# actionml/universal-recommender

Measured on NVIDIA H100. Metric: CCO train events/sec to indicator model, higher is better.
Workload: dtype int32+f64

## Files before the change

universal_recommender_b200/csrc/cco_api.cu:

```cuda
#include <cuda_runtime.h>
#include <dlfcn.h>
#include <stdarg.h>
#include <stdio.h>
#include <stdlib.h>
#include <string.h>

#include <algorithm>
#include <charconv>
#include <cmath>
#include <functional>
#include <cub/cub.cuh>
#include <nvtx3/nvToolsExt.h>
#include <condition_variable>
#include <mutex>
#include <string>
#include <thread>
#include <unordered_map>
#include <vector>

#include "../../include/cco_b200.h"
#include "cco_kernels.cuh"
#include "cco_sampler.cuh"
#include "cco_format.cuh"
#include "cco_strings.cuh"
// ... 518 lines not shown
    if (raw[i].n_rows > 0 && hist_fits_smem(c, raw[i].n_cols)) fit.push_back(i);
  for (size_t b0 = 0; b0 < fit.size(); b0 += kHistSegs) {
    const size_t b1 = std::min(fit.size(), b0 + kHistSegs);
    HistBatch hb{};
    long long nnz_sum = 0;
    int32_t max_cols = 0;
    for (size_t t = b0; t < b1; ++t) {
      nnz_sum += raw[fit[t]].nnz;
      max_cols = std::max(max_cols, raw[fit[t]].n_cols);
    }
    const size_t smem = ((size_t)max_cols + 1) / 2 * 4;
    const int per_sm = std::max(1, std::min<int>(2048 / kHistThreads, (int)(c->smem_optin / std::max<size_t>(smem + 1024, 1))));
    const long long target = (long long)c->sm_count * per_sm;
    for (size_t t = b0; t < b1; ++t) {
      const int i = fit[t];
      if (ready) CK(cudaStreamWaitEvent(s, ready[i], 0));
      const long long share = nnz_sum > 0 ? (target * raw[i].nnz + nnz_sum - 1) / nnz_sum : 1;
      const long long need = (raw[i].nnz + kHistMinEntries - 1) / kHistMinEntries;
      HistSeg &g = hb.seg[hb.n++];
      g.col = raw[i].col + raw[i].q_base;
      g.rp = raw[i].rp;
      g.nnz = raw[i].nnz;
      g.n_rows = raw[i].n_rows;
      g.q_lo = raw[i].q_base;
      g.q_hi = raw[i].q_base + raw[i].nnz;
      g.counts = counts + col_off[i];
      g.verdict = verdict ? verdict + 2 * i : nullptr;
      g.n_cols = raw[i].n_cols;
      g.cta0 = hb.cta_end;
      hb.cta_end += (int32_t)std::max(1LL, std::min(share, need));
    }
    CK(cudaFuncSetAttribute(k_col_counts_smem, cudaFuncAttributeMaxDynamicSharedMemorySize, (int)smem));
    k_col_counts_smem<<<hb.cta_end, kHistThreads, smem, s>>>(hb);
    c->launches++;
  }
  for (int i = 0; i < n_mats && copies; ++i) {
    if (raw[i].n_rows == 0 || hist_fits_smem(c, raw[i].n_cols)) continue;
    if (ready) CK(cudaStreamWaitEvent(s, ready[i], 0));
    int *v = verdict ? verdict + 2 * i : nullptr;
    if (v) {
      k_check_row_ptr<<<grid_for(raw[i].n_rows, 256, c->sm_count), 256, 0, s>>>(raw[i].n_rows, raw[i].rp, raw[i].q_base, raw[i].q_base + raw[i].nnz, v);
      c->launches++;
    }
    if (raw[i].nnz > 0) {
      k_col_histogram_flat<true><<<grid_for(raw[i].nnz, 256, c->sm_count), 256, 0, s>>>(raw[i].nnz, raw[i].col + raw[i].q_base, raw[i].n_cols,
                                                                                       counts + col_off[i], kHistCopies, copy_stride, v);
      c->launches++;
    }
  }
  if (copies) {
    k_sum_copies<<<grid_for(total_cols, 256, c->sm_count), 256, 0, s>>>(total_cols, kHistCopies, copy_stride, counts);
    c->launches++;
  }
  if (ready)
    for (int i = 0; i < n_mats; ++i) CK(cudaStreamWaitEvent(s, ready[i], 0));
  return CCO_OK;
}

static int nccl_check(int rc, const char *what) {
  if (rc != 0) return set_error(CCO_E_NCCL, "%s: %s", what, g_nccl.GetErrorString(rc));
  return CCO_OK;
}

static int downsample_all(cco_ctx *c, Arena &ar, const std::vector<DevRaw> &raw, const int *d_check , long long U,
                          const int32_t *raw_counts, int32_t *marg_all, const std::vector<long long> &col_off,
                          const cco_indicator_params_t *params, int32_t seed, uint32_t flags, std::vector<DevMat> &dm,
                          const cudaEvent_t *stage_ev ) {
  cudaStream_t s = c->stream;
  const int W = c->world, r = c->rank, n_mats = (int)raw.size();
  const long long S = (U + W - 1) / W;
  std::vector<uint32_t *> kept(n_mats, nullptr);
  std::vector<SampleScratch> sc(n_mats);
  for (int i = 0; i < n_mats; ++i) {
    DevMat *out = &dm[i];
    out->n_rows = U;
    out->n_cols = raw[i].n_cols;
    out->marg = marg_all + col_off[i];
    CKR(ar.alloc(&kept[i], (size_t)(W * S + 1)));
    CKR(ar.alloc(&out->rp, U + 1));
    CK(cudaMemsetAsync(kept[i], 0, sizeof(uint32_t) * (size_t)(W * S + 1), s));
    CKR(sample_scratch(c, ar, raw[i], raw_counts + col_off[i], params[i].max_interactions, &sc[i]));
    launch_count(c, raw[i], sc[i], params[i].max_interactions, seed, flags, d_check + 2 * i, kept[i], out->marg);
  }
  CK(cudaEventRecord(stage_ev[0], s));
  if (W > 1) {
    if (S > 0) {
      g_nccl.GroupStart();
      for (int i = 0; i < n_mats; ++i) {
        int rc = g_nccl.AllGather(kept[i] + (size_t)r * S, kept[i], (size_t)S, kNcclUint32, c->comm, s);
        if (rc != 0) { g_nccl.GroupEnd(); return nccl_check(rc, "ncclAllGather(kept counts)"); }
      }
      CKR(nccl_check(g_nccl.GroupEnd(), "ncclGroupEnd(kept counts)"));
    }
    if (col_off[n_mats] > 0)
      CKR(nccl_check(g_nccl.AllReduce(marg_all, marg_all, (size_t)col_off[n_mats], kNcclInt32, kNcclSum, c->comm, s), "ncclAllReduce(marginals)"));
  }
  std::vector<uint32_t> edge((size_t)n_mats * (W + 1), 0);
  for (int i = 0; i < n_mats; ++i) {
    CKR(exclusive_sum(c, ar, kept[i], dm[i].rp, U + 1));
    ar.release(kept[i]);
    if (W > 1)
      for (int q = 0; q <= W; ++q) CKR(mail_fetch(c, &edge[(size_t)i * (W + 1) + q], dm[i].rp + std::min<long long>((long long)q * S, U), 4));
  }
  CK(cudaEventRecord(stage_ev[1], s));
  if (W > 1) CKR(mail_wait(c));
  std::vector<long long> cap(n_mats, 0);
  std::vector<int32_t *> gathered(n_mats, nullptr);
  for (int i = 0; i < n_mats; ++i) {
    if (W == 1) {
      CKR(ar.alloc(&dm[i].col, std::max<long long>(raw[i].nnz, 1)));
      CKR(launch_write(c, ar, raw[i], sc[i], dm[i].col));
    } else {
      for (int q = 0; q < W; ++q) cap[i] = std::max<long long>(cap[i], (long long)edge[(size_t)i * (W + 1) + q + 1] - edge[(size_t)i * (W + 1) + q]);
      CKR(ar.alloc(&dm[i].col, std::max<long long>(edge[(size_t)i * (W + 1) + W], 1)));
      if (cap[i] > 0) {
        CKR(ar.alloc(&gathered[i], (size_t)(cap[i] * W)));
        CKR(launch_write(c, ar, raw[i], sc[i], gathered[i] + (size_t)r * cap[i]));
      }
    }
    ar.release(sc[i].col_thr);
    ar.release(sc[i].keep);
  }
  CK(cudaEventRecord(stage_ev[2], s));
  if (W > 1) {
    g_nccl.GroupStart();
    for (int i = 0; i < n_mats; ++i) {
      if (!gathered[i]) continue;
      int rc = g_nccl.AllGather(gathered[i] + (size_t)r * cap[i], gathered[i], (size_t)cap[i], kNcclInt32, c->comm, s);
      if (rc != 0) { g_nccl.GroupEnd(); return nccl_check(rc, "ncclAllGather(column blocks)"); }
    }
    CKR(nccl_check(g_nccl.GroupEnd(), "ncclGroupEnd(column blocks)"));
    for (int i = 0; i < n_mats; ++i) {
      if (!gathered[i]) continue;
      dim3 grid((unsigned)std::max(1, std::min(c->sm_count * 8 / W, 1024)), (unsigned)W);
      k_pack_blocks<<<grid, 256, 0, s>>>(W, S, U, cap[i], dm[i].rp, gathered[i], dm[i].col);
      c->launches++;
      ar.release(gathered[i]);
    }
  }
  CK(cudaEventRecord(stage_ev[3], s));
  CK(cudaGetLastError());
  return CCO_OK;
}


struct BinCfg {
  int group;
  int slots;
  int cap;
  int cbuf;
  int caux, keep_max, final_max;
  bool dense;
  bool bitmap;
  int bm_words;
  size_t region;
  size_t smem;
  int ctas_per_sm;
};

static int next_pow2(int x) {
  int p = 1;
  while (p < x) p <<= 1;
  return p;
}

template <int GROUP>
static int launch_rows_t(cco_ctx *c, const RowArgs &a, BinCfg &cfg, cudaStream_t st) {
  constexpr int CTA = GROUP == 32 ? 64 : GROUP;
  int occ = 1;
  void (*kern)(const RowArgs) = cfg.dense ? k_rows<GROUP, true> : k_rows<GROUP, false>;
  if constexpr (GROUP == 512 || GROUP == 256)
    if (cfg.bitmap) kern = k_rows<GROUP, false, true>;
  CK(cudaFuncSetAttribute(kern, cudaFuncAttributeMaxDynamicSharedMemorySize, (int)cfg.smem));
  CK(cudaOccupancyMaxActiveBlocksPerMultiprocessor(&occ, kern, CTA, cfg.smem));
  kern<<<c->sm_count * std::max(occ, 1) * 4, CTA, cfg.smem, st>>>(a);
  cfg.ctas_per_sm = occ;
  c->launches++;
  CK(cudaGetLastError());
  return CCO_OK;
}
static int launch_rows(cco_ctx *c, const RowArgs &a, BinCfg &cfg, cudaStream_t st) {
  switch (cfg.group) {
    case 1024: return launch_rows_t<1024>(c, a, cfg, st);
    case 512: return launch_rows_t<512>(c, a, cfg, st);
    case 256: return launch_rows_t<256>(c, a, cfg, st);
    case 128: return launch_rows_t<128>(c, a, cfg, st);
    case 32: return launch_rows_t<32>(c, a, cfg, st);
  }
  return set_error(CCO_E_INVALID_ARG, "internal: bad bin config");
}

static BinCfg make_cfg(cco_ctx *c, int group, int want_slots, int top_k, int n_cols_b) {
  BinCfg f;
  const int groups = group == 32 ? 2 : 1;
  f.group = group;
  f.final_max = next_pow2(top_k);
  f.cbuf = next_pow2(top_k + std::max(group, 128) + (group == 32 ? 64 : 0));
  if (group == 32 && top_k + 32 <= 96) f.cbuf = 128;
  f.keep_max = std::max(f.final_max, (f.cbuf - group) / 2);
  f.caux = group == 32 ? 0 : f.keep_max;
  size_t fixed = (size_t)(f.cbuf + f.caux) * 16 + 2 * 256 + 512 + 1024 + (size_t)(group / 32) * 256;
  size_t avail = (c->smem_optin - 1024) / groups;
  int max_slots = (int)((avail - fixed) / 4) & ~1023;
  f.slots = std::min(want_slots, max_slots);
  f.cap = f.slots / 2;
  f.dense = n_cols_b <= f.slots;
  f.bitmap = false;
  f.bm_words = 0;
  f.region = (fixed + (size_t)f.slots * 4 + 15) & ~(size_t)15;
  f.smem = f.region * groups;
  f.ctas_per_sm = 1;
  return f;
}

static bool use_bitmap(BinCfg &f, uint32_t max_w, int top_k, int n_cols_b) {
  if (f.dense || (f.group != 512 && f.group != 256)) return false;
  const long long seg = 32LL * (f.group / 32);
  const long long rep = (std::max<long long>(max_w, 64) + seg - 1) / seg * seg;
  const long long bm = ((long long)n_cols_b + 31) / 32;
  if (rep + bm + top_k > f.slots) return false;
  f.bitmap = true;
  f.slots = (int)rep;
  f.bm_words = (int)bm;
  return true;
}

static double llr_error_bound(long long n_users) {
  const double n = (double)n_users;
  return n > 1.0 ? std::ldexp(n * std::log(n), -47) : 0.0;
}
static bool cut_exact(long long n_users, int32_t max_marg_a, int32_t max_marg_b) {
  const double n = (double)n_users, r = (double)max_marg_a, c = (double)max_marg_b;
  if (r <= 0.0 || c <= 0.0) return true;
  double g = 2.0 / std::min(r * c, 0.5 * n);
  const double d = n - c - r + 1.0;
  if (d > 0.0) g = std::max(g, 2.0 * (1.0 / c - (r - 1.0) / d));
  return g > 2.0 * llr_error_bound(n_users);
}

struct IndicatorState {
  int mail_group = -1;
  long long rec[7] = {0, 0, 0, 0, 0, 0, 0};
  cudaEvent_t packed = nullptr;
  long long *out_ptr = nullptr;
  int32_t *p_col = nullptr, *p_cnt = nullptr;
  double *p_llr = nullptr;
  int32_t n_items_a = 0, n_cols_b = 0;
  bool emit_all = false;
};

static int enqueue_indicator(cco_ctx *c, Arena &ar, const uint32_t *at_ptr, const int32_t *at_users, int32_t n_items_a,
                             const int32_t *marg_a, int32_t max_marg_a, int32_t max_marg_b, const DevMat &B, long long n_users,
                             bool self, const cco_indicator_params_t &prm, uint32_t flags, bool emit_all, cudaEvent_t inputs_ready,
                             cudaEvent_t ev_begin, cudaEvent_t ev_end, IndicatorState *st) {
  cudaStream_t s = c->stream;
  const int32_t n_cols_b = B.n_cols;
  const int rank = c->rank, world = c->world;
  st->n_items_a = n_items_a;
  st->n_cols_b = n_cols_b;
  st->emit_all = emit_all;
  uint32_t *row_work, *masked, *sorted_work;
  unsigned long long *work64;
  long long *work_prefix;
  int32_t *ids, *rows_sorted, *d_pb = nullptr;
  size_t sort_tb = 0, order_tb = 0;
  if (n_items_a > 0)
    CK(cub::DeviceRadixSort::SortPairsDescending(nullptr, sort_tb, (const uint32_t *)nullptr, (uint32_t *)nullptr, (const int32_t *)nullptr,
                                                 (int32_t *)nullptr, n_items_a, 0, 32, s));
  int cb_bits = 1;
  while ((1LL << cb_bits) <= (long long)max_marg_b) ++cb_bits;
  cub::DoubleBuffer<uint32_t> order_cb(nullptr, nullptr);
  cub::DoubleBuffer<int32_t> order_id(nullptr, nullptr);
  if (n_cols_b > 0) CK(cub::DeviceRadixSort::SortPairs(nullptr, order_tb, order_cb, order_id, n_cols_b, 0, cb_bits, s));
  const bool beside = inputs_ready && ar.c && ((size_t)n_items_a + 1) * 8 <= Arena::kSlabMax && sort_tb <= Arena::kSlabMax &&
                      (size_t)n_cols_b * 4 <= Arena::kSlabMax && order_tb <= Arena::kSlabMax &&
                      ((size_t)max_marg_b + 2) * 4 <= Arena::kSlabMax;
  cudaStream_t ss = beside ? c->sched_stream : s;
  if (beside) CK(cudaStreamWaitEvent(ss, inputs_ready, 0));
  CKR(ar.alloc(&row_work, n_items_a + 1));
  CKR(ar.alloc(&masked, n_items_a + 1));
  CKR(ar.alloc(&work64, n_items_a + 1));
  CKR(ar.alloc(&work_prefix, n_items_a + 1));
  CKR(ar.alloc(&ids, n_items_a + 1));
  CKR(ar.alloc(&sorted_work, n_items_a + 1));
  CKR(ar.alloc(&rows_sorted, n_items_a + 1));
  CK(cudaMemsetAsync(work64 + n_items_a, 0, 8, ss));
  k_row_work<<<grid_for((long long)n_items_a * kSG, 256, c->sm_count), 256, 0, ss>>>(n_items_a, at_ptr, at_users, B.rp,
                                                                                  row_work, work64, ids, nullptr);
  c->launches++;
  CKR(exclusive_sum(c, ar, (const long long *)work64, work_prefix, (long long)n_items_a + 1, ss));
  if (world > 1) {
    CKR(ar.alloc(&d_pb, world + 1));
    k_partition_rows<<<1, ((world + 1 + 31) / 32) * 32, 0, ss>>>(work_prefix, n_items_a, world, d_pb);
    c->launches++;
  }
  k_mask_work<<<grid_for(n_items_a, 256, c->sm_count), 256, 0, ss>>>(n_items_a, row_work, d_pb, rank, masked);
  c->launches++;
  if (n_items_a > 0) {
    void *tmp;
    CKR(ar.alloc((char **)&tmp, sort_tb));
    CK(cub::DeviceRadixSort::SortPairsDescending(tmp, sort_tb, masked, sorted_work, ids, rows_sorted, n_items_a, 0, 32, ss));
    ar.release(tmp);
  }
  const int k_eff = emit_all ? 1 : prm.top_k;
  const bool warp_ok = k_eff + 32 <= 256;
  struct BinSpec { int group, slots; uint32_t max_w; };
  std::vector<BinSpec> spec = {{1024, 1 << 20, 0xffffffffu}, {1024, 1 << 20, 0xffffffffu}, {512, 16384, 8192u}, {256, 8192, 4096u}};
  if (warp_ok) {
    spec.push_back({128, 4096, 2048u});
    spec.push_back({32, 2048, 1024u});
    spec.push_back({32, 1024, 512u});
    spec.push_back({32, 512, 256u});
  } else {
    spec.push_back({128, 4096, 2048u});
  }
  const int kBins = (int)spec.size();
  std::vector<BinCfg> cfgs(kBins);
  for (int b = 0; b < kBins; ++b) cfgs[b] = make_cfg(c, spec[b].group, spec[b].slots, k_eff, n_cols_b);
  BinCfg &cfgL = cfgs[1];
  int key_bits = 1;
  while (((1LL << key_bits) - 1) <= (long long)n_cols_b) ++key_bits;
  int count_bits = 32 - key_bits;
  const long long k11_max = std::min<long long>(max_marg_a, max_marg_b);
  if (count_bits < 1 || k11_max >= (1LL << count_bits))
    return set_error(CCO_E_UNSUPPORTED,
                     "co-occurrence counts up to %lld over %d columns do not fit the packed 32-bit accumulator word "
                     "(key %d bits + count %d bits): lower maxItemsPerUser/maxEventsPerEventType for this event type "
                     "(\"Limits\" in include/cco_b200.h)", k11_max, n_cols_b, key_bits, count_bits);
  std::vector<uint32_t> h_thr(kBins);
  for (int b = 0; b < kBins; ++b) {
    const BinCfg &f = cfgs[std::min(b + 1, kBins - 1)];
    uint32_t lim = b + 1 < kBins ? spec[b + 1].max_w : 0u;
    if (b + 1 < kBins && !f.dense) lim = std::min<uint32_t>(lim, (uint32_t)f.cap);
    h_thr[b] = lim;
    if (b > 0) h_thr[b] = std::min(h_thr[b], h_thr[b - 1]);
  }
  const bool bitmap_ok = !emit_all && cut_exact(n_users, max_marg_a, max_marg_b) &&
                         2ull * (unsigned long long)std::max(max_marg_a, 0) * (unsigned long long)std::max(max_marg_b, 0) <
                             (unsigned long long)n_users;
  for (int b = 1; b < kBins && bitmap_ok; ++b) use_bitmap(cfgs[b], h_thr[b - 1], k_eff, n_cols_b);
  int32_t *d_bounds;
  CKR(ar.alloc(&d_bounds, kBins + 3));
  BinThresholds bt;
  memset(&bt, 0, sizeof bt);
  for (int b = 0; b < kBins; ++b) bt.t[b] = h_thr[b];
  k_bin_bounds<<<1, 32, 0, ss>>>(n_items_a, sorted_work, kBins, bt, d_bounds);
  c->launches++;
  int32_t *key_of_col, *first_key_of_cb, *order_id0, *order_id1;
  uint32_t *order_cb0, *order_cb1;
  const int32_t n_order = std::max<int32_t>(n_cols_b, 1);
  CKR(ar.alloc(&key_of_col, n_order));
  CKR(ar.alloc(&first_key_of_cb, (size_t)max_marg_b + 2));
  CKR(ar.alloc(&order_cb0, n_order));
  CKR(ar.alloc(&order_cb1, n_order));
  CKR(ar.alloc(&order_id0, n_order));
  CKR(ar.alloc(&order_id1, n_order));
  order_cb = cub::DoubleBuffer<uint32_t>(order_cb0, order_cb1);
  order_id = cub::DoubleBuffer<int32_t>(order_id0, order_id1);
  if (n_cols_b > 0) {
    k_col_order_init<<<grid_for(n_cols_b, 256, c->sm_count, 4), 256, 0, ss>>>(n_cols_b, B.marg, order_cb0, order_id0);
    void *tmp;
    CKR(ar.alloc((char **)&tmp, order_tb));
    CK(cub::DeviceRadixSort::SortPairs(tmp, order_tb, order_cb, order_id, n_cols_b, 0, cb_bits, ss));
    ar.release(tmp);
    k_col_order<<<grid_for(n_cols_b, 256, c->sm_count, 4), 256, 0, ss>>>(n_cols_b, max_marg_b, order_cb.Current(), order_id.Current(),
                                                                        key_of_col, first_key_of_cb);
    k_relabel_cols<<<c->sm_count * 8, 256, 0, ss>>>(B.rp + B.n_rows, key_of_col, B.col);
    c->launches += 3;
  }
  const int32_t *marg_key = reinterpret_cast<const int32_t *>(order_cb.Current()), *col_of_key = order_id.Current();
  if (beside) {
    cudaEvent_t scheduled;
    CKR(pooled_event(c, false, &scheduled));
    CK(cudaEventRecord(scheduled, ss));
    CK(cudaStreamWaitEvent(s, scheduled, 0));
  }
  ColTerm *col_terms;
  CKR(ar.alloc(&col_terms, std::max<int32_t>(n_cols_b, 1)));
  if (n_cols_b > 0) {
    k_col_terms<<<grid_for(n_cols_b, 256, c->sm_count, 4), 256, 0, s>>>(n_cols_b, marg_key, col_of_key, n_users, flags, col_terms);
    c->launches++;
  }
  int32_t stride = emit_all ? n_cols_b : std::min<int32_t>(prm.top_k, n_cols_b);
  if (stride < 1) stride = 1;
  int32_t *o_col, *o_cnt, *o_len;
  double *o_llr = nullptr;
  unsigned long long *d_distinct;
  int *d_err;
  size_t cells = (size_t)std::max(n_items_a, 1) * stride;
  CKR(ar.alloc(&o_col, cells));
  CKR(ar.alloc(&o_cnt, cells));
  if (!emit_all) CKR(ar.alloc(&o_llr, cells));
  CKR(ar.alloc(&o_len, n_items_a + 1));
  CKR(ar.alloc(&d_distinct, 2));
  CKR(ar.alloc(&d_err, 1));
  CK(cudaMemsetAsync(o_len, 0, sizeof(int32_t) * ((size_t)n_items_a + 1), s));
  CK(cudaMemsetAsync(d_distinct, 0, 16, s));
  CK(cudaMemsetAsync(d_err, 0, 4, s));
  RowArgs a;
  memset(&a, 0, sizeof a);
  a.at_ptr = at_ptr;
  a.at_users = at_users;
  a.b_ptr = B.rp;
  a.b_col = B.col;
  a.marg_a = marg_a;
  a.marg_b = marg_key;
  a.key_of_col = key_of_col;
  a.first_key_of_cb = first_key_of_cb;
  a.key_shift = 0;
  while (((long long)std::max(n_cols_b - 1, 0) >> a.key_shift) >= kCutBins) ++a.key_shift;
  a.max_marg_b = max_marg_b;
  a.col_terms = col_terms;
  a.rows_sorted = rows_sorted;
  a.row_work = row_work;
  a.bin_bounds = d_bounds;
  a.n_cols_b = n_cols_b;
  a.n_users = n_users;
  a.self = self ? 1 : 0;
  a.top_k = k_eff;
  a.has_min_llr = prm.has_min_llr;
  a.min_llr = prm.min_llr;
  a.cut_ok = cut_exact(n_users, max_marg_a, max_marg_b) ? 1 : 0;
  a.llr_eps2 = 2.0 * llr_error_bound(n_users);
  a.flags = flags;
  a.count_bits = count_bits;
  a.out_stride = stride;
  a.out_col = o_col;
  a.out_llr = o_llr;
  a.out_cnt = o_cnt;
  a.out_len = o_len;
  a.stat_distinct = d_distinct;
  a.stat_evaluated = d_distinct + 1;
  a.err_flag = d_err;
  a.emit_all = emit_all ? 1 : 0;
  if (ev_begin) CK(cudaEventRecord(ev_begin, s));
  if (n_items_a > 0) {
    CK(cudaEventRecord(c->bin_ev[8], s));
    for (int b = 0; b < kBins; ++b) {
      if (b == 0 && cfgL.dense) continue;
      RowArgs ab = a;
      ab.bin = b;
      ab.slots = cfgs[b].slots;
      ab.cap = cfgs[b].cap;
      ab.tsize_x16 = 32;
      ab.cbuf = cfgs[b].cbuf;
      ab.caux = cfgs[b].caux;
      ab.keep_max = cfgs[b].keep_max;
      ab.final_max = cfgs[b].final_max;
      ab.group_smem_bytes = (int32_t)cfgs[b].region;
      ab.bm_words = cfgs[b].bm_words;
      CK(cudaStreamWaitEvent(c->bin_stream[b], c->bin_ev[8], 0));
      CKR(launch_rows(c, ab, cfgs[b], c->bin_stream[b]));
      CK(cudaEventRecord(c->bin_ev[b], c->bin_stream[b]));
      CK(cudaStreamWaitEvent(s, c->bin_ev[b], 0));
    }
  }
  if (ev_end) CK(cudaEventRecord(ev_end, s));
  long long *len64, *rec_d;
  CKR(ar.alloc(&len64, n_items_a + 1));
  CKR(ar.alloc(&st->out_ptr, n_items_a + 1));
  CKR(ar.alloc(&rec_d, 8));
  k_len_to_i64<<<grid_for((long long)n_items_a + 1, 256, c->sm_count), 256, 0, s>>>(n_items_a, o_len, d_pb, rank, len64);
  c->launches++;
  CKR(exclusive_sum(c, ar, len64, st->out_ptr, (long long)n_items_a + 1));
  CKR(ar.alloc(&st->p_col, cells));
  if (!(flags & CCO_FLAG_RESULT_NO_COUNT) || emit_all) CKR(ar.alloc(&st->p_cnt, cells));
  if (!emit_all && !(flags & CCO_FLAG_RESULT_NO_LLR)) CKR(ar.alloc(&st->p_llr, cells));
  if (n_items_a > 0) {
    k_compact_rows<<<grid_for((long long)n_items_a * 32, 256, c->sm_count), 256, 0, s>>>(n_items_a, stride, st->out_ptr, o_col, o_llr,
                                                                                      o_cnt, st->p_col, st->p_llr, st->p_cnt);
    c->launches++;
  }
  k_indicator_record<<<1, 32, 0, s>>>(n_items_a, d_pb, rank, st->out_ptr, work_prefix, d_distinct, d_err, rec_d);
  c->launches++;
  CKR(mail_fetch(c, st->rec, rec_d, sizeof(long long) * 7));
  CKR(mail_close(c, &st->mail_group));
  if (!st->packed) CK(cudaEventCreateWithFlags(&st->packed, cudaEventDisableTiming));
  CK(cudaEventRecord(st->packed, s));
  CK(cudaGetLastError());
  for (void *p : {(void *)o_col, (void *)o_cnt, (void *)o_llr, (void *)len64})
    if (p) ar.release(p);
  return CCO_OK;
}

struct IndicatorOut {
  int64_t row_begin = 0, row_end = 0;
  int64_t nnz = 0;
  int64_t products = 0, distinct = 0, evaluated = 0;
};

static int finish_indicator(cco_ctx *c, IndicatorState *st, uint32_t flags, int index, ResultMat *rm, IndicatorOut *io) {
  CKR(mail_wait_group(c, st->mail_group));
  const int32_t lo = (int32_t)st->rec[0], hi = (int32_t)st->rec[1];
// ... 5945 lines not shown
```

universal_recommender_b200/csrc/cco_kernels.cuh:

```cuda
#pragma once

#include <cuda_runtime.h>
#include <stdint.h>

namespace cco {

struct RowArgs {
  const uint32_t *at_ptr;
  const int32_t *at_users;
  const uint32_t *b_ptr;
  const int32_t *b_col;
  const int32_t *marg_a;
  const int32_t *marg_b;
  const int32_t *key_of_col;
  const int32_t *first_key_of_cb;
  int32_t key_shift;
  const uint2 *ext;
  int32_t max_marg_b;
  const int32_t *rows_sorted;
  const uint32_t *row_work;
  const int32_t *bin_bounds;
  int32_t bin;
  int32_t n_cols_b;
  long long n_users;
// ... 414 lines not shown
        if (gtid >= d) incl += v;
      }
      const int excl = incl - ssum, need = k - above;
      if (excl < need && need <= incl) {
        int run = excl;
#pragma unroll
        for (int j = 0; j < 8; ++j) {
          if (run < need && run + c[j] >= need) { ctrl[24] = 255 - 8 * gtid - j; ctrl[25] = run; ctrl[26] = c[j]; }
          run += c[j];
        }
      }
    }
    group_sync<GROUP>();
    const int D = vc[24], c_gt = vc[25], c_d = vc[26];
    if (wi == 0) pre0 |= (uint32_t)D << sh; else if (wi == 1) pre1 |= (uint32_t)D << sh; else pre2 |= (uint32_t)D << sh;
    nb += 8;
    kept = above + c_gt + c_d;
    if (kept <= M || nb == 96) break;
    above += c_gt;
    group_sync<GROUP>();
  }
  if (gtid == 0) ctrl[27] = 0;
  group_sync<GROUP>();
  if (GROUP == 32) {
    int w = 0;
    for (int i0 = 0; i0 < n; i0 += 32) {
      const int i = i0 + gtid;
      uint4 e = make_uint4(0u, 0u, 0u, 0u);
      bool keep = false;
      if (i < n) {
        e = tk[i];
        const uint32_t w0 = e.y, w1 = e.x, w2 = ~e.z;
        keep = w0 > pre0 || (w0 == pre0 && (w1 > pre1 || (w1 == pre1 && w2 >= pre2)));
      }
      const unsigned m = __ballot_sync(0xffffffffu, keep);
      __syncwarp();
      if (keep) tk[w + __popc(m & ((1u << gtid) - 1u))] = e;
      w += __popc(m);
      __syncwarp();
    }
  } else {
    for (int i = gtid; i < n; i += GROUP) {
      const uint4 e = tk[i];
      const uint32_t w0 = e.y, w1 = e.x, w2 = ~e.z;
      const bool keep = w0 > pre0 || (w0 == pre0 && (w1 > pre1 || (w1 == pre1 && w2 >= pre2)));
      if (keep) aux[atomicAdd(&ctrl[27], 1)] = e;
    }
    group_sync<GROUP>();
    for (int i = gtid; i < kept; i += GROUP) tk[i] = aux[i];
  }
  if (gtid == 0) {
    ctrl[0] = kept;
    ctrl[4] = (int)pre1; ctrl[5] = (int)pre0; ctrl[6] = (int)~pre2; ctrl[7] = 0;
    ctrl[1] = 1;
  }
  group_sync<GROUP>();
  return kept;
}

constexpr int kCutBins = 512;
constexpr int kDomLevels = 15;
constexpr int kX12N = 31;

__device__ __forceinline__ void cut_find(const uint32_t *h1, uint32_t need, int lane, int *ctrl) {
  uint32_t sum = 0;
  for (int wi = 0; wi < 8; ++wi) { const uint32_t v = h1[lane * 8 + wi]; sum += (v & 0xffffu) + (v >> 16); }
  uint32_t incl = sum;
#pragma unroll
  for (int d = 1; d < 32; d <<= 1) {
    const uint32_t v = __shfl_up_sync(0xffffffffu, incl, d);
    if (lane >= d) incl += v;
  }
  const uint32_t excl = incl - sum;
  int found = 0x7fffffff;
  uint32_t below = 0;
  if (excl < need && incl >= need) {
    uint32_t run = excl;
    for (int wi = 0; wi < 8; ++wi) {
      const uint32_t v = h1[lane * 8 + wi];
      if (run + (v & 0xffffu) >= need) { found = lane * 16 + 2 * wi; below = run; break; }
      run += v & 0xffffu;
      if (run + (v >> 16) >= need) { found = lane * 16 + 2 * wi + 1; below = run; break; }
      run += v >> 16;
    }
  }
#pragma unroll
  for (int o = 16; o > 0; o >>= 1) {
    found = min(found, __shfl_xor_sync(0xffffffffu, found, o));
    below = max(below, __shfl_xor_sync(0xffffffffu, below, o));
  }
  if (lane == 0) { ctrl[9] = found; ctrl[10] = (int)below; }
}

template <int GROUP, bool DENSE>
__device__ __forceinline__ void accumulate(uint32_t *table, uint32_t tsize, uint32_t b, int cbits, uint32_t n_pass,
                                           uint32_t pass, int *err_flag) {
  if (DENSE) {
    atomicAdd(&table[b], 1u);
    return;
  }
  if (n_pass > 1 && ((b * 0x85ebca6bu) >> 12) % n_pass != pass) return;
  uint32_t slot = __umulhi(b * 0x9e3779b1u, tsize);
  const uint32_t want = b << cbits;
  uint32_t probes = 0;
  while (true) {
    const uint32_t w = *reinterpret_cast<volatile uint32_t *>(&table[slot]);
    if ((w >> cbits) == b && w != kEmpty) { atomicAdd(&table[slot], 1u); return; }
    if (w == kEmpty) {
      const uint32_t old = atomicCAS(&table[slot], kEmpty, want | 1u);
      if (old == kEmpty) return;
      if ((old >> cbits) == b) { atomicAdd(&table[slot], 1u); return; }
    }
    slot = (slot + 1 == tsize) ? 0 : slot + 1;
    if (++probes > tsize) { atomicOr(err_flag, 1); return; }
  }
}

template <int GROUP, bool DENSE, bool BITMAP>
__device__ __forceinline__ void count_window(const RowArgs &a, uint32_t *table, uint32_t *seen, uint32_t tsize, int cbits,
                                             uint32_t n_pass, uint32_t pass, uint32_t off, uint32_t s, uint32_t p_lo,
                                             uint32_t p_hi, int lane) {
  for (uint32_t p0 = p_lo; p0 < p_hi; p0 += 64) {
    uint32_t bb[2];
    bool act[2];
#pragma unroll
    for (int h = 0; h < 2; ++h) {
      const uint32_t p = p0 + h * 32 + lane;
      int j = 0;
#pragma unroll
      for (int st = 16; st > 0; st >>= 1) {
        const int c = j + st;
        const uint32_t v = __shfl_sync(0xffffffffu, off, c);
        if (v <= p) j = c;
      }
      const uint32_t sj = __shfl_sync(0xffffffffu, s, j), oj = __shfl_sync(0xffffffffu, off, j);
      act[h] = p < p_hi;
      bb[h] = act[h] ? (uint32_t)a.b_col[sj + (p - oj)] : 0u;
    }
    if (BITMAP) {
      uint32_t old[2];
#pragma unroll
      for (int h = 0; h < 2; ++h) old[h] = act[h] ? atomicOr(&seen[bb[h] >> 5], 1u << (bb[h] & 31u)) : 0u;
#pragma unroll
      for (int h = 0; h < 2; ++h)
        if (act[h] && ((old[h] >> (bb[h] & 31u)) & 1u)) accumulate<GROUP, false>(table, tsize, bb[h], cbits, 1u, 0u, a.err_flag);
    } else {
#pragma unroll
      for (int h = 0; h < 2; ++h)
        if (act[h]) accumulate<GROUP, DENSE>(table, tsize, bb[h], cbits, n_pass, pass, a.err_flag);
    }
  }
}

template <int GROUP>
struct RowsMinBlocks {
  static constexpr int value = GROUP == 512 ? 2 : GROUP == 256 ? 4 : GROUP == 128 ? 8 : GROUP == 32 ? 12 : 1;
};

template <int GROUP, bool DENSE, bool BITMAP = false>
__global__ void __launch_bounds__(GROUP == 32 ? 64 : GROUP, RowsMinBlocks<GROUP>::value) k_rows(const RowArgs a) {
  static_assert(!BITMAP || (GROUP > 32 && !DENSE), "bitmap rows are CTA-owned rows of a hashed bin");
  const int GROUPS = GROUP == 32 ? (int)(blockDim.x >> 5) : 1;
  constexpr int NW = GROUP / 32;
  extern __shared__ __align__(16) unsigned char smem_raw[];
  const int tid = threadIdx.x, lane = tid & 31;
  const int gid = tid / GROUP, gtid = tid % GROUP, gw = gtid >> 5;
  unsigned char *base = smem_raw + (size_t)gid * a.group_smem_bytes;
  uint4 *tk = reinterpret_cast<uint4 *>(base);
  uint4 *aux = tk + a.cbuf;
  double *x12tab = reinterpret_cast<double *>(aux + a.caux);
  double *x11tab = x12tab + 32;
  int *ctrl = reinterpret_cast<int *>(x11tab + 32);
  int *hist = ctrl + 128;
  uint32_t *wqueue = reinterpret_cast<uint32_t *>(hist + 256);
  uint32_t *h1 = reinterpret_cast<uint32_t *>(hist);
  uint32_t *table = wqueue + NW * 64;
  uint32_t *seen = table + a.slots;
  uint32_t *singles = seen + a.bm_words;
  volatile int *vctrl = ctrl;

  const int row_begin = a.bin_bounds[a.bin], row_end = a.bin_bounds[a.bin + 1];
  const bool varargs = (a.flags & CCO_FLAG_ENTROPY_VARARGS) != 0;
  const int cbits = a.count_bits;
  const uint32_t cmask = (1u << cbits) - 1u;
  const int prune_limit = a.cbuf - GROUP;
  const long long N = a.n_users;
  const double xN = xlogx(N);
  unsigned long long distinct_local = 0, evaluated_local = 0;
  if (gtid < 32) x11tab[gtid] = xlogx((long long)gtid);

  for (int ri = row_begin + blockIdx.x * GROUPS + gid; ri < row_end; ri += gridDim.x * GROUPS) {
    const int item = a.rows_sorted[ri];
    const uint32_t u_begin = a.at_ptr[item], u_end = a.at_ptr[item + 1];
    const long long ra = a.marg_a[item];
    const int diag = a.self ? a.key_of_col[item] : -1;
    const bool keyed = 2ull * (unsigned long long)ra * (unsigned long long)a.max_marg_b < (unsigned long long)N;
    uint32_t n_pass = 1, tsize = (uint32_t)a.n_cols_b;
    if (!DENSE) {
      const uint32_t w = a.row_work[item];
      const uint32_t dcells = BITMAP ? w / 2u : w;
      const uint32_t dbound = dcells < (uint32_t)a.n_cols_b ? dcells : (uint32_t)a.n_cols_b;
      n_pass = BITMAP ? 1u : (dbound + (uint32_t)a.cap - 1u) / (uint32_t)a.cap;
      if (n_pass == 0) n_pass = 1;
      tsize = n_pass > 1 ? (uint32_t)a.slots
                         : (uint32_t)min((unsigned long long)a.slots,
                                         max(((unsigned long long)dbound * (unsigned long long)a.tsize_x16) >> 4, 64ull));
      tsize = min((uint32_t)a.slots, (tsize + 32u * NW - 1u) / (32u * NW) * (32u * NW));
    }
    group_sync<GROUP>();
    if (gtid < 32) {
      const long long v = (gtid < kX12N) ? ra - gtid : N - ra;
      x12tab[gtid] = v >= 0 ? xlogx(v) : 0.0;
    }
    if (gtid == 0) { ctrl[0] = 0; ctrl[1] = 0; }
    if (gtid < 16) ctrl[40 + gtid] = 0x7fffffff;
    int emitted = 0;

    for (uint32_t pass = 0; pass < n_pass; ++pass) {
      for (uint32_t i = gtid; i < tsize; i += GROUP) table[i] = DENSE ? 0u : kEmpty;
      if (BITMAP)
        for (int i = gtid; i < a.bm_words; i += GROUP) seen[i] = 0u;
      group_sync<GROUP>();
      if (NW == 1) {
        for (uint32_t c0 = u_begin; c0 < u_end; c0 += 32) {
          const uint32_t i = c0 + lane;
          uint32_t s = 0, len = 0;
          if (i < u_end) {
            const int32_t u = a.at_users[i];
            s = a.b_ptr[u];
            len = a.b_ptr[u + 1] - s;
          }
          uint32_t off = len;
#pragma unroll
          for (int d = 1; d < 32; d <<= 1) {
            const uint32_t v = __shfl_up_sync(0xffffffffu, off, d);
            if (lane >= d) off += v;
          }
          const uint32_t total = __shfl_sync(0xffffffffu, off, 31);
          off = i < u_end ? off - len : 0xffffffffu;
          count_window<GROUP, DENSE, BITMAP>(a, table, seen, tsize, cbits, n_pass, pass, off, s, 0u, total, lane);
        }
      } else {
        uint2 *wofs = reinterpret_cast<uint2 *>(wqueue);
        int *wsum = hist;
        for (uint32_t w0 = u_begin; w0 < u_end; w0 += GROUP) {
          const uint32_t nwin = min((uint32_t)GROUP, u_end - w0);
          uint32_t s = 0, len = 0;
          if ((uint32_t)gtid < nwin) {
            const int32_t u = a.at_users[w0 + gtid];
            s = a.b_ptr[u];
            len = a.b_ptr[u + 1] - s;
          }
          uint32_t incl = len;
#pragma unroll
          for (int d = 1; d < 32; d <<= 1) {
            const uint32_t v = __shfl_up_sync(0xffffffffu, incl, d);
            if (lane >= d) incl += v;
          }
          if (lane == 31) wsum[gw] = (int)incl;
          __syncthreads();
          uint32_t wpre = lane < NW ? (uint32_t)wsum[lane] : 0u;
#pragma unroll
          for (int d = 1; d < NW; d <<= 1) {
            const uint32_t v = __shfl_up_sync(0xffffffffu, wpre, d);
            if (lane >= d) wpre += v;
          }
          const uint32_t T = __shfl_sync(0xffffffffu, wpre, NW - 1);
          const uint32_t before = gw == 0 ? 0u : __shfl_sync(0xffffffffu, wpre, gw - 1);
          wofs[gtid] = make_uint2(s, before + incl - len);
          __syncthreads();
          const uint32_t p_lo = (uint32_t)((unsigned long long)T * gw / NW);
          const uint32_t p_hi = (uint32_t)((unsigned long long)T * (gw + 1) / NW);
          if (p_lo < p_hi) {
            uint32_t lo = 0, hi = nwin - 1;
            while (lo < hi) {
              const uint32_t mid = (lo + hi + 1) >> 1;
              if (wofs[mid].y <= p_lo) lo = mid; else hi = mid - 1;
            }
            for (uint32_t j0 = lo, p = p_lo; p < p_hi; j0 += 32) {
              const uint2 e = j0 + lane < nwin ? wofs[j0 + lane] : make_uint2(0u, 0xffffffffu);
              const uint32_t wend = min(p_hi, j0 + 32 < nwin ? wofs[j0 + 32].y : T);
              count_window<GROUP, DENSE, BITMAP>(a, table, seen, tsize, cbits, n_pass, pass, e.y, e.x, p, wend, lane);
              p = wend;
            }
          }
          __syncthreads();
        }
      }
      group_sync<GROUP>();
      const uint32_t seg = (((tsize + NW - 1) / NW) + 31u) & ~31u;
      const uint32_t seg_lo = min((uint32_t)gw * seg, tsize), seg_hi = min(seg_lo + seg, tsize);
      uint32_t n_mine = 0;
      for (uint32_t pos = seg_lo; pos < seg_hi; pos += 32) {
        const uint32_t idx = pos + lane;
        uint32_t w = DENSE ? 0u : kEmpty;
        if (idx < seg_hi) w = table[idx];
        const bool valid = DENSE ? (w != 0u) : (w != kEmpty);
        const uint32_t word = DENSE ? ((idx << cbits) | w) : w;
        const unsigned m = __ballot_sync(0xffffffffu, valid);
        __syncwarp();
        if (valid) {
          table[seg_lo + n_mine + __popc(m & ((1u << lane) - 1u))] = BITMAP ? word + 1u : word;
          if (BITMAP) atomicAnd(&seen[(word >> cbits) >> 5], ~(1u << ((word >> cbits) & 31u)));
        }
        n_mine += __popc(m);
        __syncwarp();
      }
      if (lane == 0) distinct_local += n_mine;
      uint32_t n_list = n_mine;
      const uint32_t *singles_mine = singles;
      if (BITMAP) {
        group_sync<GROUP>();
        if (gtid == 0 && diag >= 0) {
          const uint32_t bit = 1u << ((uint32_t)diag & 31u);
          if (seen[diag >> 5] & bit) {
            seen[diag >> 5] &= ~bit;
            ++distinct_local;
          }
        }
        group_sync<GROUP>();
        const uint32_t nbw = (uint32_t)a.bm_words, per = (nbw + GROUP - 1u) / GROUP;
        const uint32_t w_lo = min((uint32_t)gtid * per, nbw), w_hi = min(w_lo + per, nbw);
        uint32_t cnt = 0;
        for (uint32_t i = w_lo; i < w_hi; ++i) cnt += __popc(seen[i]);
        distinct_local += cnt;
        uint32_t incl = cnt;
#pragma unroll
        for (int d = 1; d < 32; d <<= 1) {
          const uint32_t v = __shfl_up_sync(0xffffffffu, incl, d);
          if (lane >= d) incl += v;
        }
        int *wsum = hist;
        if (lane == 31) wsum[gw] = (int)incl;
        __syncthreads();
        uint32_t wpre = lane < NW ? (uint32_t)wsum[lane] : 0u;
#pragma unroll
        for (int d = 1; d < NW; d <<= 1) {
          const uint32_t v = __shfl_up_sync(0xffffffffu, wpre, d);
          if (lane >= d) wpre += v;
        }
        const uint32_t total = __shfl_sync(0xffffffffu, wpre, NW - 1);
        const uint32_t before = gw == 0 ? 0u : __shfl_sync(0xffffffffu, wpre, gw - 1);
        const uint32_t n_single = min(total, (uint32_t)a.top_k);
        uint32_t o = before + incl - cnt;
        for (uint32_t i = w_lo; i < w_hi && o < n_single; ++i)
          for (uint32_t m = seen[i]; m != 0u && o < n_single; m &= m - 1u)
            singles[o++] = (((i << 5) | (uint32_t)(__ffs(m) - 1)) << cbits) | 1u;
        __syncthreads();
        const uint32_t s_lo = (uint32_t)((unsigned long long)n_single * gw / NW);
        const uint32_t s_hi = (uint32_t)((unsigned long long)n_single * (gw + 1) / NW);
        singles_mine = singles + s_lo;
        n_list = n_mine + (s_hi - s_lo);
      }
      if (!BITMAP && a.emit_all) {
        int basepos = 0;
        if (lane == 0) basepos = atomicAdd(&ctrl[0], (int)n_mine);
        basepos = __shfl_sync(0xffffffffu, basepos, 0);
        for (uint32_t q = lane; q < n_mine; q += 32) {
          const uint32_t word = table[seg_lo + q];
          const size_t o = (size_t)item * a.out_stride + emitted + basepos + q;
          a.out_col[o] = a.col_terms[word >> cbits].col;
          a.out_cnt[o] = (int32_t)(word & cmask);
        }
        group_sync<GROUP>();
        emitted += vctrl[0];
        group_sync<GROUP>();
        if (gtid == 0) ctrl[0] = 0;
        group_sync<GROUP>();
        continue;
      }
      int cut1 = 0x7fffffff;
      if (!BITMAP && a.cut_ok && a.row_work[item] < 65536u) {
        int sh = keyed ? a.key_shift : 0, hi_sh = 32;
        uint32_t prefix = 0, need = (uint32_t)a.top_k;
        while (true) {
          for (int i = gtid; i < kCutBins / 2; i += GROUP) h1[i] = 0u;
          group_sync<GROUP>();
          for (uint32_t q0 = 0; q0 < n_mine; q0 += 32) {
            const uint32_t q = q0 + lane;
            if (q < n_mine) {
              const uint32_t word = table[seg_lo + q];
              const uint32_t b = word >> cbits;
              if ((word & cmask) == 1u && (int)b != diag) {
                uint32_t bin = kCutBins;
                if (keyed) {
                  if (((unsigned long long)(b ^ prefix) >> hi_sh) == 0) bin = (b >> sh) & (kCutBins - 1);
                } else {
                  const uint32_t cb = (uint32_t)a.marg_b[b];
                  if (cb < (uint32_t)kCutBins && 2ull * (unsigned long long)ra * cb < (unsigned long long)N) bin = cb;
                }
                if (bin < (uint32_t)kCutBins) atomicAdd(&h1[bin >> 1], 1u << (16u * (bin & 1u)));
              }
            }
          }
          group_sync<GROUP>();
          if (gtid < 32) cut_find(h1, need, lane, ctrl);
          group_sync<GROUP>();
          const int found = vctrl[9];
          if (!keyed || found == 0x7fffffff) { cut1 = found; break; }
          prefix |= (uint32_t)found << sh;
          need -= (uint32_t)vctrl[10];
          if (sh == 0) { cut1 = (int)prefix; break; }
          hi_sh = sh;
          sh = sh > 9 ? sh - 9 : 0;
        }
      }
      const double x_ra = x12tab[0], x_nra = x12tab[kX12N];
      const double row_e = varargs ? __dsub_rn(xN, __dadd_rn(__dadd_rn(0.0, x_ra), x_nra))
                                   : __dsub_rn(__dsub_rn(xN, x_ra), x_nra);
      uint32_t *wq = wqueue + gw * 64;
      uint32_t pos = 0;
      int qn = 0;
      while (true) {
        while (qn < 32 && pos < n_list) {
          const uint32_t q = pos + lane;
          bool surv = false;
          uint32_t word = 0;
          if (q < n_list) {
            word = (!BITMAP || q < n_mine) ? table[seg_lo + q] : singles_mine[q - n_mine];
            const uint32_t b = word >> cbits, k11 = word & cmask;
            if ((int)b != diag) {
              if (keyed) {
                surv = !(k11 <= (uint32_t)kDomLevels && (int)b >= vctrl[40 + k11]);
                if (k11 == 1u && (int)b > cut1) surv = false;
              } else {
                const long long cb = a.marg_b[b];
                const bool pos_side = (unsigned long long)ra * (unsigned long long)cb < (unsigned long long)k11 * (unsigned long long)N;
                surv = !(pos_side && k11 <= (uint32_t)kDomLevels && (int)cb >= vctrl[40 + k11]);
                if (k11 == 1u && (int)cb > cut1 && 2ull * (unsigned long long)ra * (unsigned long long)cb < (unsigned long long)N)
                  surv = false;
              }
            }
          }
          const unsigned m = __ballot_sync(0xffffffffu, surv);
          if (surv) wq[qn + __popc(m & ((1u << lane) - 1u))] = word;
          qn += __popc(m);
          pos += 32;
          __syncwarp();
        }
        const int take = qn < 32 ? qn : 32;
        bool pass_ok = false;
        uint4 e = make_uint4(0u, 0u, 0u, 0u);
        if (lane < take) {
          const uint32_t word = wq[qn - take + lane];
          const uint32_t b = word >> cbits, k11 = word & cmask;
          const ColTerm ct = a.col_terms[b];
          const long long cb = ct.cb;
          const bool pos_side = (unsigned long long)ra * (unsigned long long)cb < (unsigned long long)k11 * (unsigned long long)N;
          const uint32_t kf = k11 < (uint32_t)kDomLevels ? k11 : (uint32_t)kDomLevels;
          ++evaluated_local;
          const long long k21 = cb - k11, k22 = N - ra - cb + k11;
          const double x11 = k11 < 32 ? x11tab[k11] : xlogx_u32(k11);
          const double x12 = k11 < kX12N ? x12tab[k11] : xlogx_u32((uint32_t)(ra - k11));
          const double x21 = k11 == 1 ? ct.x_cbm1 : xlogx_u32((uint32_t)k21), x22 = xlogx_u32((uint32_t)k22);
          double mat_e;
          if (varargs)
            mat_e = __dsub_rn(xN, __dadd_rn(__dadd_rn(__dadd_rn(__dadd_rn(0.0, x11), x12), x21), x22));
          else
            mat_e = __dsub_rn(__dsub_rn(__dsub_rn(__dsub_rn(xN, x11), x12), x21), x22);
          const double sre = __dadd_rn(row_e, ct.col_e);
          const double v = (sre < mat_e) ? 0.0 : __dmul_rn(2.0, __dsub_rn(sre, mat_e));
          const bool min_ok = !a.has_min_llr || v >= a.min_llr;
          pass_ok = v > 0.0 && min_ok;
          const double vm = __dadd_rn(v, a.llr_eps2);
          bool strict_fail = v > 0.0 && !min_ok && vm < a.min_llr;
          const unsigned long long key = (unsigned long long)__double_as_longlong(v);
          e = make_uint4((uint32_t)key, (uint32_t)(key >> 32), (uint32_t)ct.col, k11);
          if (pass_ok && vctrl[1]) {
            const uint4 thr = make_uint4((uint32_t)vctrl[4], (uint32_t)vctrl[5], (uint32_t)vctrl[6], (uint32_t)vctrl[7]);
            pass_ok = !cand_better(thr, e);
            strict_fail = vm < __hiloint2double((int)thr.y, (int)thr.x);
          }
          if (strict_fail && pos_side) {
            const int f = keyed ? a.first_key_of_cb[cb] : (int)cb;
            for (uint32_t kk = kf; kk >= 1 && f < vctrl[40 + kk]; --kk) atomicMin(&ctrl[40 + kk], f);
          }
        }
        qn -= take;
        const unsigned m = __ballot_sync(0xffffffffu, pass_ok);
        int basepos_round = 0;
        if (m) {
          int basepos = 0;
          if (lane == 0) basepos = atomicAdd(&ctrl[0], __popc(m));
          basepos = __shfl_sync(0xffffffffu, basepos, 0);
          if (pass_ok) tk[basepos + __popc(m & ((1u << lane) - 1u))] = e;
          basepos_round = basepos;
        }
        const bool more = qn > 0 || pos < n_list;
        int mine = 0;
        if (m) mine = basepos_round + __popc(m);
        bool any_more, need_prune;
        if (GROUP == 32) {
          __syncwarp();
          any_more = more;
          need_prune = mine > prune_limit;
        } else {
          any_more = __syncthreads_or(more ? 1 : 0) != 0;
          need_prune = __syncthreads_or(mine > prune_limit ? 1 : 0) != 0;
        }
        if (need_prune) {
          const int n = vctrl[0];
          if (GROUP > 32 && n <= 512) {
            if (gw == 0) reduce_candidates<32>(tk, aux, n, a.top_k, a.keep_max, hist, ctrl, lane);
            group_sync<GROUP>();
          } else {
            reduce_candidates<GROUP>(tk, aux, n, a.top_k, a.keep_max, hist, ctrl, gtid);
          }
        }
        if (!any_more) break;
      }
      group_sync<GROUP>();
    }
    if (a.emit_all) {
      if (gtid == 0) a.out_len[item] = emitted;
    } else {
      int n = vctrl[0];
      if (n > 0) {
        if (GROUP > 32 && n <= 512) {
          if (gw == 0) {
            int m = n;
            if (m > a.final_max) m = reduce_candidates<32>(tk, aux, m, a.top_k, a.final_max, hist, ctrl, lane);
            sort_candidates<32>(tk, m, lane);
            if (lane == 0) ctrl[0] = m;
          }
          group_sync<GROUP>();
          n = vctrl[0];
        } else {
          if (n > a.final_max) n = reduce_candidates<GROUP>(tk, aux, n, a.top_k, a.final_max, hist, ctrl, gtid);
          sort_candidates<GROUP>(tk, n, gtid);
        }
        const int keep = n < a.top_k ? n : a.top_k;
        for (int i = gtid; i < keep; i += GROUP) {
          const size_t o = (size_t)item * a.out_stride + i;
          const uint4 e = tk[i];
          a.out_col[o] = (int32_t)e.z;
          a.out_llr[o] = __longlong_as_double((long long)(((unsigned long long)e.y << 32) | e.x));
          a.out_cnt[o] = (int32_t)e.w;
        }
        if (gtid == 0) a.out_len[item] = keep;
      } else if (gtid == 0) {
        a.out_len[item] = 0;
      }
    }
  }
  for (int o = 16; o > 0; o >>= 1) distinct_local += __shfl_xor_sync(0xffffffffu, distinct_local, o);
  if (lane == 0 && distinct_local) atomicAdd(a.stat_distinct, distinct_local);
  for (int o = 16; o > 0; o >>= 1) evaluated_local += __shfl_xor_sync(0xffffffffu, evaluated_local, o);
  if (lane == 0 && evaluated_local) atomicAdd(a.stat_evaluated, evaluated_local);
}

__global__ void k_compact_rows(int32_t n_items, int32_t stride, const long long *__restrict__ out_ptr,
                               const int32_t *__restrict__ col, const double *__restrict__ llr, const int32_t *__restrict__ cnt,
                               int32_t *__restrict__ p_col, double *__restrict__ p_llr, int32_t *__restrict__ p_cnt) {
  int warp = (blockIdx.x * blockDim.x + threadIdx.x) >> 5, lane = threadIdx.x & 31;
  int nwarps = (gridDim.x * blockDim.x) >> 5;
  for (int item = warp; item < n_items; item += nwarps) {
    const long long o = out_ptr[item];
    const int n = (int)(out_ptr[item + 1] - o);
    size_t src = (size_t)item * stride;
    for (int i = lane; i < n; i += 32) {
      p_col[o + i] = col[src + i];
      if (p_llr) p_llr[o + i] = llr[src + i];
      if (p_cnt) p_cnt[o + i] = cnt[src + i];
    }
  }
}

__global__ void k_expand_keys(long long n_rows, const long long *__restrict__ rp, const int32_t *__restrict__ col,
                              unsigned long long *__restrict__ keys) {
  const int lane = threadIdx.x % kSG;
  long long row = (blockIdx.x * (long long)blockDim.x + threadIdx.x) / kSG;
  const long long stride = (long long)gridDim.x * blockDim.x / kSG;
// ... 153 lines not shown
```

Measured before the change: 4.219 billion.

## Replace hash-table counting with warp radix sort for small warp-owned rows

For warp-owned (GROUP 32) hashed bins with small row work, adds a SORTED kernel variant. It gathers the co-occurring column keys into shared memory, radix-sorts them with packed 16-bit digit histograms and match_any scatter, and then run-length encodes them into (key, count) words. It also keeps only the first top_k singletons, which replaces the hash-table probe and compaction. The intent is to avoid hash collisions and table clearing and to shrink shared memory per row, which may raise occupancy. In exchange it adds multiple sort passes and bypasses the cut1 prefix pruning for these rows.

```diff
diff --git a/universal_recommender_b200/csrc/cco_api.cu b/universal_recommender_b200/csrc/cco_api.cu
--- a/universal_recommender_b200/csrc/cco_api.cu
+++ b/universal_recommender_b200/csrc/cco_api.cu
@@ -694,6 +694,7 @@
   int caux, keep_max, final_max;
   bool dense;
   bool bitmap;
+  bool sorted;
   int bm_words;
   size_t region;
   size_t smem;
@@ -713,6 +714,8 @@
   void (*kern)(const RowArgs) = cfg.dense ? k_rows<GROUP, true> : k_rows<GROUP, false>;
   if constexpr (GROUP == 512 || GROUP == 256)
     if (cfg.bitmap) kern = k_rows<GROUP, false, true>;
+  if constexpr (GROUP == 32)
+    if (cfg.sorted) kern = k_rows<32, false, false, true>;
   CK(cudaFuncSetAttribute(kern, cudaFuncAttributeMaxDynamicSharedMemorySize, (int)cfg.smem));
   CK(cudaOccupancyMaxActiveBlocksPerMultiprocessor(&occ, kern, CTA, cfg.smem));
   kern<<<c->sm_count * std::max(occ, 1) * 4, CTA, cfg.smem, st>>>(a);
@@ -748,6 +751,7 @@
   f.cap = f.slots / 2;
   f.dense = n_cols_b <= f.slots;
   f.bitmap = false;
+  f.sorted = false;
   f.bm_words = 0;
   f.region = (fixed + (size_t)f.slots * 4 + 15) & ~(size_t)15;
   f.smem = f.region * groups;
@@ -764,6 +768,20 @@
   f.bitmap = true;
   f.slots = (int)rep;
   f.bm_words = (int)bm;
+  return true;
+}
+
+static bool use_sorted(BinCfg &f, uint32_t max_w, int count_bits) {
+  constexpr int kAliased = 256 + 64;
+  if (f.dense || f.group != 32 || max_w > 1024u) return false;
+  const int slots = std::max(2 * (int)max_w - kAliased, (int)max_w);
+  const int kb = 32 - count_bits, passes = (kb + 8) / 9;
+  const int dbits = std::max((kb + passes - 1) / passes, 6);
+  if (slots > f.slots || (long long)passes << (dbits - 1) > 4LL * f.cbuf) return false;
+  f.sorted = true;
+  f.region -= (size_t)(f.slots - slots) * 4;
+  f.smem = f.region * 2;
+  f.slots = slots;
   return true;
 }
 
@@ -880,7 +898,10 @@
   const bool bitmap_ok = !emit_all && cut_exact(n_users, max_marg_a, max_marg_b) &&
                          2ull * (unsigned long long)std::max(max_marg_a, 0) * (unsigned long long)std::max(max_marg_b, 0) <
                              (unsigned long long)n_users;
-  for (int b = 1; b < kBins && bitmap_ok; ++b) use_bitmap(cfgs[b], h_thr[b - 1], k_eff, n_cols_b);
+  for (int b = 1; b < kBins && bitmap_ok; ++b) {
+    use_bitmap(cfgs[b], h_thr[b - 1], k_eff, n_cols_b);
+    use_sorted(cfgs[b], h_thr[b - 1], count_bits);
+  }
   int32_t *d_bounds;
   CKR(ar.alloc(&d_bounds, kBins + 3));
   BinThresholds bt;
diff --git a/universal_recommender_b200/csrc/cco_kernels.cuh b/universal_recommender_b200/csrc/cco_kernels.cuh
--- a/universal_recommender_b200/csrc/cco_kernels.cuh
+++ b/universal_recommender_b200/csrc/cco_kernels.cuh
@@ -590,14 +590,138 @@
   }
 }
 
+struct SortDigits {
+  int passes, dbits, hwords;
+};
+__device__ __forceinline__ SortDigits sort_digits(int cbits) {
+  const int kb = 32 - cbits;
+  SortDigits d;
+  d.passes = (kb + 8) / 9;
+  d.dbits = max((kb + d.passes - 1) / d.passes, 6);
+  d.hwords = 1 << (d.dbits - 1);
+  return d;
+}
+__device__ __forceinline__ void digit_count(uint32_t *h, const SortDigits &sd, uint32_t b) {
+  for (int p = 0; p < sd.passes; ++p) {
+    const uint32_t dg = (b >> (p * sd.dbits)) & ((1u << sd.dbits) - 1u);
+    atomicAdd(&h[p * sd.hwords + (dg >> 1)], 1u << (16u * (dg & 1u)));
+  }
+}
+
+constexpr int kGatherDepth = 4;
+__device__ __forceinline__ void gather_window(const RowArgs &a, uint32_t *keys, uint32_t *h, const SortDigits &sd, uint32_t off,
+                                              uint32_t s, uint32_t p_hi, int lane) {
+  for (uint32_t p0 = 0; p0 < p_hi; p0 += 32 * kGatherDepth) {
+    uint32_t bb[kGatherDepth];
+    bool act[kGatherDepth];
+#pragma unroll
+    for (int hh = 0; hh < kGatherDepth; ++hh) {
+      const uint32_t p = p0 + hh * 32 + lane;
+      int j = 0;
+#pragma unroll
+      for (int st = 16; st > 0; st >>= 1) {
+        const int c = j + st;
+        const uint32_t v = __shfl_sync(0xffffffffu, off, c);
+        if (v <= p) j = c;
+      }
+      const uint32_t sj = __shfl_sync(0xffffffffu, s, j), oj = __shfl_sync(0xffffffffu, off, j);
+      act[hh] = p < p_hi;
+      bb[hh] = act[hh] ? (uint32_t)a.b_col[sj + (p - oj)] : 0u;
+    }
+#pragma unroll
+    for (int hh = 0; hh < kGatherDepth; ++hh)
+      if (act[hh]) {
+        keys[p0 + hh * 32 + lane] = bb[hh];
+        digit_count(h, sd, bb[hh]);
+      }
+  }
+}
+
+__device__ __forceinline__ void digit_scan(uint32_t *h, int hwords, int lane) {
+  const int per = hwords >> 5;
+  uint32_t sum = 0;
+  for (int j = 0; j < per; ++j) { const uint32_t v = h[lane * per + j]; sum += (v & 0xffffu) + (v >> 16); }
+  uint32_t incl = sum;
+#pragma unroll
+  for (int d = 1; d < 32; d <<= 1) {
+    const uint32_t v = __shfl_up_sync(0xffffffffu, incl, d);
+    if (lane >= d) incl += v;
+  }
+  uint32_t run = incl - sum;
+  for (int j = 0; j < per; ++j) {
+    const uint32_t v = h[lane * per + j], lo = v & 0xffffu;
+    h[lane * per + j] = run | ((run + lo) << 16);
+    run += lo + (v >> 16);
+  }
+  __syncwarp();
+}
+
+__device__ uint32_t sort_runs(uint32_t *keys, uint32_t w, uint32_t *h, const SortDigits &sd, int cbits, int diag, int top_k,
+                              uint32_t *n_runs, int lane) {
+  const unsigned lt = (1u << lane) - 1u, le = (2u << lane) - 1u;
+  uint32_t *src = keys, *dst = keys + w;
+  for (int p = 0; p < sd.passes; ++p) {
+    uint32_t *hp = h + p * sd.hwords;
+    digit_scan(hp, sd.hwords, lane);
+    const int sh = p * sd.dbits;
+    for (uint32_t i0 = 0; i0 < w; i0 += 32) {
+      const uint32_t i = i0 + lane;
+      const bool valid = i < w;
+      const uint32_t k = valid ? src[i] : 0u;
+      const uint32_t dg = valid ? (k >> sh) & ((1u << sd.dbits) - 1u) : 0xffffffffu;
+      const unsigned peers = __match_any_sync(0xffffffffu, dg);
+      const uint32_t hsh = 16u * (dg & 1u);
+      const uint32_t base = valid ? (hp[dg >> 1] >> hsh) & 0xffffu : 0u;
+      __syncwarp();
+      if (valid) {
+        const uint32_t r = __popc(peers & lt);
+        dst[base + r] = k;
+        if (r == 0) atomicAdd(&hp[dg >> 1], (uint32_t)__popc(peers) << hsh);
+      }
+      __syncwarp();
+    }
+    uint32_t *t = src; src = dst; dst = t;
+  }
+  uint32_t *out = keys + w;
+  uint32_t n = 0, n_single = 0, nr = 0, prev_key = kEmpty, head_pos = 0;
+  for (uint32_t i0 = 0; i0 < w; i0 += 32) {
+    const uint32_t i = i0 + lane;
+    const bool valid = i < w;
+    const uint32_t k = valid ? src[i] : kEmpty;
+    const uint32_t nk = i + 1 < w ? src[i + 1] : kEmpty;
+    uint32_t pk = __shfl_up_sync(0xffffffffu, k, 1);
+    if (lane == 0) pk = prev_key;
+    const unsigned hm = __ballot_sync(0xffffffffu, valid && k != pk);
+    nr += __popc(hm);
+    const unsigned mine = hm & le;
+    const uint32_t hpos = mine ? i0 + 31u - (uint32_t)__clz(mine) : head_pos;
+    const uint32_t len = i + 1u - hpos;
+    const bool off_diag = valid && k != nk && (int)k != diag;
+    const bool single = off_diag && len == 1u;
+    const unsigned sm = __ballot_sync(0xffffffffu, single);
+    const bool keep = off_diag && (len > 1u || n_single + __popc(sm & lt) < (uint32_t)top_k);
+    n_single += __popc(sm);
+    const unsigned km = __ballot_sync(0xffffffffu, keep);
+    prev_key = __shfl_sync(0xffffffffu, k, 31);
+    head_pos = __shfl_sync(0xffffffffu, hpos, 31);
+    __syncwarp();
+    if (keep) out[n + __popc(km & lt)] = (k << cbits) | len;
+    n += __popc(km);
+    __syncwarp();
+  }
+  *n_runs = nr;
+  return n;
+}
+
 template <int GROUP>
 struct RowsMinBlocks {
   static constexpr int value = GROUP == 512 ? 2 : GROUP == 256 ? 4 : GROUP == 128 ? 8 : GROUP == 32 ? 12 : 1;
 };
 
-template <int GROUP, bool DENSE, bool BITMAP = false>
+template <int GROUP, bool DENSE, bool BITMAP = false, bool SORTED = false>
 __global__ void __launch_bounds__(GROUP == 32 ? 64 : GROUP, RowsMinBlocks<GROUP>::value) k_rows(const RowArgs a) {
   static_assert(!BITMAP || (GROUP > 32 && !DENSE), "bitmap rows are CTA-owned rows of a hashed bin");
+  static_assert(!SORTED || (GROUP == 32 && !DENSE && !BITMAP), "sorted rows are warp-owned rows of a hashed bin");
   const int GROUPS = GROUP == 32 ? (int)(blockDim.x >> 5) : 1;
   constexpr int NW = GROUP / 32;
   extern __shared__ __align__(16) unsigned char smem_raw[];
@@ -626,6 +750,8 @@
   const double xN = xlogx(N);
   unsigned long long distinct_local = 0, evaluated_local = 0;
   if (gtid < 32) x11tab[gtid] = xlogx((long long)gtid);
+  uint32_t *dhist = reinterpret_cast<uint32_t *>(tk);
+  const SortDigits sd = sort_digits(cbits);
 
   for (int ri = row_begin + blockIdx.x * GROUPS + gid; ri < row_end; ri += gridDim.x * GROUPS) {
     const int item = a.rows_sorted[ri];
@@ -634,7 +760,7 @@
     const int diag = a.self ? a.key_of_col[item] : -1;
     const bool keyed = 2ull * (unsigned long long)ra * (unsigned long long)a.max_marg_b < (unsigned long long)N;
     uint32_t n_pass = 1, tsize = (uint32_t)a.n_cols_b;
-    if (!DENSE) {
+    if (!DENSE && !SORTED) {
       const uint32_t w = a.row_work[item];
       const uint32_t dcells = BITMAP ? w / 2u : w;
       const uint32_t dbound = dcells < (uint32_t)a.n_cols_b ? dcells : (uint32_t)a.n_cols_b;
@@ -655,10 +781,15 @@
     int emitted = 0;
 
     for (uint32_t pass = 0; pass < n_pass; ++pass) {
-      for (uint32_t i = gtid; i < tsize; i += GROUP) table[i] = DENSE ? 0u : kEmpty;
+      if (SORTED)
+        for (int i = lane; i < sd.passes * sd.hwords; i += 32) dhist[i] = 0u;
+      else
+        for (uint32_t i = gtid; i < tsize; i += GROUP) table[i] = DENSE ? 0u : kEmpty;
       if (BITMAP)
         for (int i = gtid; i < a.bm_words; i += GROUP) seen[i] = 0u;
       group_sync<GROUP>();
+      uint32_t *keys = table + a.slots - 2u * (SORTED ? a.row_work[item] : 0u);
+      uint32_t n_keys = 0;
       if (NW == 1) {
         for (uint32_t c0 = u_begin; c0 < u_end; c0 += 32) {
           const uint32_t i = c0 + lane;
@@ -676,7 +807,12 @@
           }
           const uint32_t total = __shfl_sync(0xffffffffu, off, 31);
           off = i < u_end ? off - len : 0xffffffffu;
-          count_window<GROUP, DENSE, BITMAP>(a, table, seen, tsize, cbits, n_pass, pass, off, s, 0u, total, lane);
+          if (SORTED) {
+            gather_window(a, keys + n_keys, dhist, sd, off, s, total, lane);
+            n_keys += total;
+          } else {
+            count_window<GROUP, DENSE, BITMAP>(a, table, seen, tsize, cbits, n_pass, pass, off, s, 0u, total, lane);
+          }
         }
       } else {
         uint2 *wofs = reinterpret_cast<uint2 *>(wqueue);
@@ -729,7 +865,14 @@
       const uint32_t seg = (((tsize + NW - 1) / NW) + 31u) & ~31u;
       const uint32_t seg_lo = min((uint32_t)gw * seg, tsize), seg_hi = min(seg_lo + seg, tsize);
       uint32_t n_mine = 0;
-      for (uint32_t pos = seg_lo; pos < seg_hi; pos += 32) {
+      const uint32_t *list = table;
+      if (SORTED) {
+        uint32_t n_runs;
+        n_mine = sort_runs(keys, n_keys, dhist, sd, cbits, diag, a.top_k, &n_runs, lane);
+        list = keys + n_keys;
+        if (lane == 0) distinct_local += n_runs;
+      }
+      for (uint32_t pos = seg_lo; pos < seg_hi && !SORTED; pos += 32) {
         const uint32_t idx = pos + lane;
         uint32_t w = DENSE ? 0u : kEmpty;
         if (idx < seg_hi) w = table[idx];
@@ -744,7 +887,7 @@
         n_mine += __popc(m);
         __syncwarp();
       }
-      if (lane == 0) distinct_local += n_mine;
+      if (lane == 0 && !SORTED) distinct_local += n_mine;
       uint32_t n_list = n_mine;
       const uint32_t *singles_mine = singles;
       if (BITMAP) {
@@ -790,7 +933,7 @@
         singles_mine = singles + s_lo;
         n_list = n_mine + (s_hi - s_lo);
       }
-      if (!BITMAP && a.emit_all) {
+      if (!BITMAP && !SORTED && a.emit_all) {
         int basepos = 0;
         if (lane == 0) basepos = atomicAdd(&ctrl[0], (int)n_mine);
         basepos = __shfl_sync(0xffffffffu, basepos, 0);
@@ -808,7 +951,7 @@
         continue;
       }
       int cut1 = 0x7fffffff;
-      if (!BITMAP && a.cut_ok && a.row_work[item] < 65536u) {
+      if (!BITMAP && !SORTED && a.cut_ok && a.row_work[item] < 65536u) {
         int sh = keyed ? a.key_shift : 0, hi_sh = 32;
         uint32_t prefix = 0, need = (uint32_t)a.top_k;
         while (true) {
@@ -855,7 +998,7 @@
           bool surv = false;
           uint32_t word = 0;
           if (q < n_list) {
-            word = (!BITMAP || q < n_mine) ? table[seg_lo + q] : singles_mine[q - n_mine];
+            word = (!BITMAP || q < n_mine) ? list[seg_lo + q] : singles_mine[q - n_mine];
             const uint32_t b = word >> cbits, k11 = word & cmask;
             if ((int)b != diag) {
               if (keyed) {
```

New measurement: 4.445 billion, median of 6. 5.3% higher.
